# rlvc/FEALESS

Measured on AMD Instinct MI355X. Metric: frames/sec (640x480 RGB-D x N templates, 20 ICP iters), higher is better.
Workload: dtype u8

## Files before the change

fealess_amd/csrc/fl_icp.hip:

```cpp
#include "fl_internal.h"
#include <float.h>
#include <math.h>
#include <string.h>
#include <type_traits>
#include <mutex>
#include <map>
#include <utility>

#define ICP_BS_SMALL 256
#define ICP_BS_WIDE 1024
#define ICP_DT 512
#ifdef FL_ICP_PHASES
#define TSTAMP(k) do { if (threadIdx.x == 0) { long long now_ = clock64(); S.tacc[k] += now_ - S.tlast; S.tlast = now_; } } while (0)
#define CH_STAMP_BEGIN long long c_add = 0, c_bar = 0, c_last = clock64()
#define CH_STAMP(v) { const long long now_ = clock64(); v += now_ - c_last; c_last = now_; }
#define CH_STAMP_END(k) { if (threadIdx.x == 0) { S.hist[k] += (unsigned)(c_add >> 4); S.hist[(k) + 1] += (unsigned)(c_bar >> 4); } }
#define PR_STAMP_BARRIER(k, every) { const long long b0_ = clock64(); tile_barrier(); if (threadIdx.x == 64) S.hist[k] += (unsigned)(((clock64() - b0_) * (every)) >> 4); }
#define ST_STAMP_BEGIN long long st_acc[6] = {0, 0, 0, 0, 0, 0}, st_last = clock64()
#define ST_STAMP(k) { const long long now_ = clock64(); st_acc[k] += now_ - st_last; st_last = now_; }
#define ST_ARRIVED(a, b) asm volatile("" :: "v"(a), "v"(b));
#define ST_STAMP_END { if ((threadIdx.x & 63) == 0) for (int k = 0; k < 5; ++k) atomicAdd(&S.stime[k], (unsigned long long)st_acc[k]); }
#else
#define TSTAMP(k) do { } while (0)
#define CH_STAMP_BEGIN
#define CH_STAMP(v) { }
#define CH_STAMP_END(k) { }
#define PR_STAMP_BARRIER(k, every) tile_barrier()
#define ST_STAMP_BEGIN
#define ST_STAMP(k) { }
#define ST_ARRIVED(a, b)
#define ST_STAMP_END
#endif
__device__ __forceinline__ void tile_barrier()
{
  __builtin_amdgcn_s_waitcnt(0xC07F);
  __builtin_amdgcn_s_barrier();
}
#define ICP_PARITY_WPE 4
#define ICP_FAST_WPE 4
#define ICP_PLANE_WPE 4
#define ICP_MODE_WPE(MODE) ((MODE) == FL_ICP_PARITY ? ICP_PARITY_WPE : ((MODE) == FL_ICP_POINT_TO_PLANE ? ICP_PLANE_WPE : ICP_FAST_WPE))
#define ICP_NBQ 4
#define ICP_NBUF_SMALL 4
#define ICP_TILE_W 16
#define ICP_BMACRO 4
#define ICP_STAGE_CAP 384
#define ICP_NB 10

struct IcpWsLayout {
  size_t ref, mod, sref, zimg, nn, bnd, nd, dterm, perm, cell_start, cell_cur, nrm, total;
  int ncell_max;
};
static __host__ __device__ inline size_t al256(size_t v) { return (v + 255) & ~(size_t)255; }
static __host__ __device__ inline IcpWsLayout icp_layout(int n)
{
  IcpWsLayout L;
  size_t o = 0, nn = (size_t)(n > 0 ? n : 1);
  L.ncell_max = n + 4096;
  L.ref = o; o = al256(o + 12 * nn);
  L.mod = o; o = al256(o + 12 * nn);
  L.sref = o; o = al256(o + 16 * (nn + 4));
  L.zimg = o; o = al256(o + 4 * (nn + 4));
  L.nn = o; o = al256(o + 4 * nn);
  L.bnd = o; o = al256(o + 4 * nn);
  L.nd = o; o = al256(o + 4 * nn);
  L.dterm = o; o = al256(o + 4 * nn + 4 * ICP_DT);
  L.perm = o; o = al256(o + 4 * nn);
  L.cell_start = o; o = al256(o + 4 * ((size_t)L.ncell_max + 1));
  L.cell_cur = o; o = al256(o + 4 * (size_t)L.ncell_max);
  L.nrm = o; o = al256(o + 12 * nn);
  L.total = o;
  return L;
}
size_t fl_icp_ws_bytes(int n_pts_max) { return icp_layout(n_pts_max).total; }

struct IcpJob {
// ... 22 lines not shown
  const uint16_t *scene_base;
  size_t scene_stride;
  const FlPyrInfo *pyr;
  const int *class_first;
  const float *poses;
  const uint16_t *const *depth_ptrs;
  fl_recognition_result *results;
  const FlRefineJob *jobs;
  const int *order;
};

template <int BS_>
struct IcpSharedT {
  static constexpr int BS = BS_;
  static constexpr int NW = BS_ / 64;
  static constexpr int NPROD = NW >= 8 ? NW - NW / 4 : NW - 1;
  static constexpr int CHAIN_NBUF = BS_ >= 1024 ? 4 : ICP_NBUF_SMALL;
  static constexpr int TQ = NPROD * 64;
  int cw;
  __device__ __forceinline__ int producer_slot() const
  {
    const int t = (int)threadIdx.x, w = t >> 6;
    if (NW >= 8) return (w & 3) == 0 ? -1 : t - 64 * (1 + (w >> 2));
    const int v = (w - __builtin_amdgcn_readfirstlane(cw) - 1) & (NW - 1);
    return v == NW - 1 ? -1 : v * 64 + (t & 63);
  }
  __device__ __forceinline__ int chain_lane() const
  {
    const int t = (int)threadIdx.x;
    if (NW >= 8) return t < 64 ? t : -1;
    return (t >> 6) == __builtin_amdgcn_readfirstlane(cw) ? (t & 63) : -1;
  }
  static constexpr int TS = TQ + 4;
  float R[9], T[3], Ropt[9], Topt[3];
  float dist_mean, dist_diff, px, thr;
  int iter, n_corr, go, ok;
  int cnt, inl;
  int stop;
  int a1_next;
  float xmin, ymin, inv_c;
  int GX, GY, nsorted;
  float sums[16];
  double dsum[NW][32];
  int iscan[NW + 1];
  int iscan2[2][NW];
  float fred[4][NW];
  int n, rect_m[4], rect_r[4], status, g;
  alignas(16) float prod[2][15][TS];
  static constexpr bool BSUM = NW >= 8;
  alignas(16) float dtile[2][TQ];
  static constexpr int STAGE_FLOATS = NW * 384 * 4, TILE_FLOATS = 2 * 15 * TS + 2 * TQ;
  alignas(16) float stage_pad[STAGE_FLOATS > TILE_FLOATS ? STAGE_FLOATS - TILE_FLOATS : 4];
  alignas(16) float dchain[2][ICP_DT];
#ifdef FL_ICP_PHASES
  long long tacc[16], tlast, tkernel;
  long long wall0;
  unsigned long long stime[8];
  unsigned hist[40];
#endif
};

__device__ __forceinline__ bool vvalid(float z) { return z <= 900.0f; }
__device__ __forceinline__ float uniform_f(float v) { return __int_as_float(__builtin_amdgcn_readfirstlane(__float_as_int(v))); }
__device__ __forceinline__ int cvt_i32_sat(float f)
{
  int r;
  asm("v_cvt_i32_f32 %0, %1" : "=v"(r) : "v"(f));
  return r;
}

#include "fl_icp_search.h"

template <class SH>
__device__ __forceinline__ int block_sum_int(SH &S, int v)
{
#pragma unroll
  for (int s = 32; s >= 1; s >>= 1) v += __shfl_xor(v, s, 64);
  __syncthreads();
  if ((threadIdx.x & 63) == 0) S.iscan[threadIdx.x >> 6] = v;
  __syncthreads();
  int t = 0;
#pragma unroll
  for (int i = 0; i < SH::NW; ++i) t += S.iscan[i];
  return t;
}

__device__ __forceinline__ double shfl_xor_d(double v, int s)
{
  int lo = __double2loint(v), hi = __double2hiint(v);
  lo = __shfl_xor(lo, s, 64);
  hi = __shfl_xor(hi, s, 64);
  return __hiloint2double(hi, lo);
}

template <int NS, class SH>
__device__ __forceinline__ void block_sum_double(SH &S, double *v)
{
  const int lane = threadIdx.x & 63, wave = threadIdx.x >> 6;
#pragma unroll
  for (int k = 0; k < NS; ++k) {
    double x = v[k];
#pragma unroll
    for (int s = 32; s >= 1; s >>= 1) x += shfl_xor_d(x, s);
    v[k] = x;
  }
  __syncthreads();
  if (lane == 0)
    for (int k = 0; k < NS; ++k) S.dsum[wave][k] = v[k];
  __syncthreads();
  if (threadIdx.x < NS) {
    double t = 0;
// ... 418 lines not shown
  for (int a = 0; a < 6; ++a) A[a][a] += 1.0e-12 * tr;
  for (int c = 0; c < 6 && ok; ++c) {
    double d = A[c][c];
    for (int k = 0; k < c; ++k) d -= A[c][k] * A[c][k];
    if (!(d > 1.0e-13 * tr)) { ok = false; break; }
    d = sqrt(d);
    A[c][c] = d;
    for (int r = c + 1; r < 6; ++r) {
      double v = A[r][c];
      for (int k = 0; k < c; ++k) v -= A[r][k] * A[c][k];
      A[r][c] = v / d;
    }
  }
  if (ok) {
    for (int r = 0; r < 6; ++r) {
      double v = x[r];
      for (int k = 0; k < r; ++k) v -= A[r][k] * x[k];
      x[r] = v / A[r][r];
    }
    for (int r = 5; r >= 0; --r) {
      double v = x[r];
      for (int k = r + 1; k < 6; ++k) v -= A[k][r] * x[k];
      x[r] = v / A[r][r];
    }
    const double wx = x[0], wy = x[1], wz = x[2], t2 = wx * wx + wy * wy + wz * wz, t = sqrt(t2);
    const double sa = t > 1.0e-9 ? sin(t) / t : 1.0 - t2 / 6.0, sb = t > 1.0e-9 ? (1.0 - cos(t)) / t2 : 0.5 - t2 / 24.0;
    const double Kx[9] = {0, -wz, wy, wz, 0, -wx, -wy, wx, 0};
    for (int i = 0; i < 3; ++i)
      for (int j = 0; j < 3; ++j) {
        double k2 = 0;
        for (int k = 0; k < 3; ++k) k2 += Kx[i * 3 + k] * Kx[k * 3 + j];
        S.Ropt[i * 3 + j] = (float)((i == j ? 1.0 : 0.0) + sa * Kx[i * 3 + j] + sb * k2);
      }
    for (int k = 0; k < 3; ++k) S.Topt[k] = (float)x[3 + k];
  }
  S.ok = ok && finite_all(S.Ropt, 9) && finite_all(S.Topt, 3);
}
template <class SH>
__device__ __forceinline__ void pose_accumulate(SH &S)
{
  float RT[3];
  mat_vec(S.Ropt, S.T, RT);
  for (int k = 0; k < 3; ++k) S.T[k] = RT[k] + S.Topt[k];
  mat_mat(S.Ropt, S.R, S.R);
}
__device__ __forceinline__ void icp_result_none(fl_icp_result *res)
{
  for (int i = 0; i < 9; ++i) res->R[i] = 0.f;
  for (int i = 0; i < 3; ++i) res->T[i] = 0.f;
  res->dist_mean = -1.0f; res->px_ratio = 0.f;
  res->iters = 0; res->n_corr_last = 0;
}

template <class IDX>
__device__ __forceinline__ int nn_get(IDX v) { return sizeof(IDX) == 2 && (int)v == 0xFFFF ? -1 : (int)v; }
template <int MODE, bool ORG, class IDX, class SH>
__device__ __forceinline__ void icp_run(SH &S, uint8_t *wsb, const IcpWsLayout &L, int n_ref, int n_model,
                        int it_thr, float dmt, float ddt, fl_icp_result *res, const OrgGeom &og)
{
  constexpr int BS = SH::BS, NW = SH::NW;
  float *ref = (float *)(wsb + L.ref), *mod = (float *)(wsb + L.mod);
  float4 *sref = (float4 *)(wsb + L.sref);
  const float *jsrc = ORG ? (const float *)sref : ref;
  const int *idximg = ORG ? (const int *)((const uint8_t *)sref + org_idximg_offset(og.cw * og.ch)) : nullptr;
  constexpr bool IDX16 = sizeof(IDX) == 2;
  static_assert(!IDX16 || (MODE == FL_ICP_PARITY && ORG && SH::NW < 8), "16-bit indices: the 256-thread parity kernel of the organised search only");
  IDX *nn = (IDX *)(wsb + L.nn);
  bnd_t *bnd = (bnd_t *)(wsb + L.bnd);
  float *nd = (float *)(wsb + L.nd), *dterm = (float *)(wsb + L.dterm);
  const IDX *perm = (const IDX *)(wsb + L.perm);
  const uint16_t *pix = (const uint16_t *)(wsb + L.dterm);
  const float *zref = (const float *)(wsb + L.nd);
  const float *nrm = (const float *)(wsb + L.nrm);
  int *cell_start = (int *)(wsb + L.cell_start), *cell_cur = (int *)(wsb + L.cell_cur);
  constexpr bool plane = MODE == FL_ICP_POINT_TO_PLANE;
  constexpr int NSUM = plane ? 27 : 15;

  if (threadIdx.x == 0) {
    for (int i = 0; i < 9; ++i) S.R[i] = 0.f;
    for (int i = 0; i < 3; ++i) S.T[i] = 0.f;
    S.iter = 0;
    S.n_corr = 0;
    S.px = 0.f;
#ifdef FL_ICP_PHASES
    for (int i = 0; i < 16; ++i) S.tacc[i] = 0;
    for (int i = 0; i < 40; ++i) S.hist[i] = 0;
    for (int i = 0; i < 8; ++i) S.stime[i] = 0;
    S.tlast = clock64();
    S.tacc[6] = S.tlast - S.tkernel;
#endif
  }
  __syncthreads();
  if (n_model < 3 || n_ref < 3 || n_ref < n_model) {
    if (threadIdx.x == 0) icp_result_none(res);
    __syncthreads();
    return;
  }
  if (!ORG) build_grid(S, ref, n_ref, sref, cell_start, cell_cur, L.ncell_max);
  TSTAMP(0);
  for (int i = threadIdx.x; i < n_model; i += BS)
    if (!vvalid(mod[3 * i + 2])) { mod[3 * i] = 0.f; mod[3 * i + 1] = 0.f; mod[3 * i + 2] = 0.f; }
  if (threadIdx.x == 0) {
    S.R[0] = S.R[4] = S.R[8] = 1.f;
    S.dist_diff = FLT_MAX;
  }
  __syncthreads();
  constexpr bool SPEC = BS >= ICP_BS_WIDE && MODE == FL_ICP_PARITY && ORG;
  static_assert(!(IDX16 && SPEC), "pix[] / zref[] live where the deferred chain keeps dterm[] / nd[]");
  float mean_ub = l2dist_phase<MODE, SPEC, false>(S, mod, ref, bnd, dterm, n_model, FLT_MAX, nullptr, nullptr, pix, zref, og);
  int pending = SPEC ? 1 : 0;
  bool have_nn = false;
  float old_mean = 0.0f;

  const auto ctx = org_search_ctx(mod, bnd, perm, (const float *)sref, (const float *)(wsb + L.zimg), n_model, og);
  auto chain_and_search = [&](const int pend, const bool want, const float r_lim, const float old_mean_) {
    if (pend && threadIdx.x < 64) {
      const float acc = chain_deferred<SH::CHAIN_NBUF>(dterm, S.dchain, n_model);
      if (threadIdx.x == 0) {
        const int counter = S.cnt, inl = S.inl;
        float dm = acc;
        if (counter > 0) dm /= (float)inl;
        const float new_mean = counter > 0 ? dm : FLT_MAX;
        S.px = counter > 0 ? (float)inl / (float)counter : 0.0f;
        if (pend == 2) {
          S.dist_diff = old_mean_ - new_mean;
          pose_accumulate(S);
        }
        S.dist_mean = new_mean;
        const bool go = (new_mean > dmt) && (S.dist_diff > ddt) && (S.iter < it_thr);
        *(volatile int *)&S.stop = go ? 0 : 1;
      }
    }
    if (want)
      org_search<SH, SPEC>(S, ctx, r_lim, true, [&](bool active, int i, float, float, float, int j, float d) {
        if (active) {
          nn[i] = (IDX)j;
          nd[i] = d;
          if (j >= 0) bnd_st(bnd, i, sqrt_upper(d));
        }
      });
  };

  for (;;) {
    if (SPEC) {
      const int it_done = __builtin_amdgcn_readfirstlane(S.iter);
      const bool want = !have_nn && it_done >= 1 && it_done < it_thr;
      if (pending || want) {
        const float r_lim = pending ? sqrtf(3.0f * mean_ub) * 1.00001f : sqrtf(3 * S.dist_mean);
        if (threadIdx.x == 0) { S.a1_next = 0; S.stop = 0; }
        __syncthreads();
        chain_and_search(pending, want, uniform_f(r_lim), old_mean);
        __syncthreads();
        TSTAMP(2);
        if (want) have_nn = true;
        pending = 0;
      }
    }
    if (threadIdx.x == 0) S.go = (S.dist_mean > dmt) && (S.dist_diff > ddt) && (S.iter < it_thr);
    __syncthreads();
    if (!S.go) break;
    if (threadIdx.x == 0) { ++S.iter; S.thr = plane ? (3 * S.dist_mean) * (3 * S.dist_mean) : 3 * S.dist_mean; S.a1_next = 0; }
    __syncthreads();
// ... 18 lines not shown
#pragma unroll
          for (int b = a; b < 6; ++b) ds[q++] += J[a] * J[b];
#pragma unroll
        for (int a = 0; a < 6; ++a) ds[21 + a] += J[a] * e;
      } else if (!parity) {
        const float m[3] = {m0, m1, m2}, r[3] = {r0, r1, r2};
#pragma unroll
        for (int a = 0; a < 3; ++a)
#pragma unroll
          for (int b = 0; b < 3; ++b) ds[a * 3 + b] += (double)m[a] * (double)r[b];
#pragma unroll
        for (int q = 0; q < 3; ++q) { ds[9 + q] += (double)m[q]; ds[12 + q] += (double)r[q]; }
      }
    };
    if (!index_pairs && !SPEC) {
      const float r_thr = uniform_f(sqrtf(thr));
      auto on_found = [&](bool active, int i, float qx, float qy, float qz, int j, float d) {
        const bool keep = d <= thr;
        if (active) {
          nn[i] = (IDX)(keep ? j : -1);
          if (j >= 0) bnd_st(bnd, i, sqrt_upper(d));
        }
        if (keep) {
          ++kept;
          if (!parity) { const F3 rv = ld3_u32(jsrc, j); pair_sums(qx, qy, qz, rv.x, rv.y, rv.z, j); }
        }
      };
      if (ORG) {
        if (MODE == FL_ICP_PARITY && NW < 8) org_search_pipe(S, ctx, r_thr, on_found);
        else org_search<SH, SPEC>(S, ctx, r_thr, false, on_found);
      } else {
        const NnGrid G = nn_grid(S);
        int i = threadIdx.x;
        float qx = 0.f, qy = 0.f, qz = 0.f, qb = 0.f;
        if (i < n_model) { const F3 q3 = ld3_u32(mod, i); qx = q3.x; qy = q3.y; qz = q3.z; qb = bnd_ld(bnd, i); }
        for (; i < n_model; i += BS) {
          const int in = min(i + BS, n_model - 1);
          const F3 nq3 = ld3_u32(mod, in);
          const float nqx = nq3.x, nqy = nq3.y, nqz = nq3.z, nqb = bnd_ld(bnd, in);
          int j = -1;
          float d = NAN;
          if (thr >= 0.f && isfinite(qx) && isfinite(qy) && isfinite(qz))
            nn_search_grid(G, sref, cell_start, qx, qy, qz, nn_radius(qx, qy, qz, fminf(qb, r_thr)), &j, &d);
          on_found(true, i, qx, qy, qz, j, d);
          qx = nqx; qy = nqy; qz = nqz; qb = nqb;
        }
      }
      __syncthreads();
      TSTAMP(2);
    }
    constexpr int TQ = parity ? SH::TQ : BS;
    const int slot = parity ? S.producer_slot() : (int)threadIdx.x;
    const int clane = parity ? S.chain_lane() : -1;
    const int ntiles = (parity || index_pairs) ? (rows + TQ - 1) / TQ : 0;
    float acc = 0.0f;
    if (parity && iter > 1) {
      struct Row {
        int j;
        float d;
        bool in;
        F3 m, r;
      };
      constexpr bool ZIMG = ORG && NW < 8;
      const float *zimg = (const float *)(wsb + L.zimg);
      const float inv_cw = uniform_f(1.0f / (float)max(og.cw, 1));
      auto row_load = [&](Row &w, int t) {
        const int i = t * TQ + slot;
        w.in = i < rows;
        const int ic = min(i, rows - 1);
        w.j = ld_u32(nn, ic);
        w.d = SPEC ? ld_u32(nd, ic) : 0.0f;
        w.m = ld3_u32(mod, ic);
      };
      auto row_gather = [&](Row &w) {
        if (!(w.in && (!SPEC || w.d <= thr)) || (IDX16 && w.j == 0xFFFF)) w.j = -1;
        if (ZIMG) w.r.x = ld_u32(zimg, max(w.j, 0));
        else w.r = ld3_u32(jsrc, max(w.j, 0));
      };
      auto row_write = [&](const Row &w, int t) {
        const bool have = w.j >= 0;
        if (SPEC && have) ++kept;
        float (*tile)[SH::TS] = S.prod[t & 1];
        F3 rp = w.r;
        if (ZIMG) {
          const int jj = max(w.j, 0);
          int vv, uu;
          if (ctx.small_crop) {
            vv = (int)(((float)jj + 0.5f) * inv_cw);
            uu = jj - __mul24(vv, og.cw);
            if (uu < 0) { --vv; uu += og.cw; } else if (uu >= og.cw) { ++vv; uu -= og.cw; }
          } else {
            vv = jj / og.cw;
            uu = jj - vv * og.cw;
          }
          rp = org_point(og, uu, vv, w.r.x);
        }
        const float mm[3] = {have ? w.m.x : 0.0f, have ? w.m.y : 0.0f, have ? w.m.z : 0.0f};
        const float rr[3] = {have ? rp.x : 0.0f, have ? rp.y : 0.0f, have ? rp.z : 0.0f};
#pragma unroll
        for (int a = 0; a < 3; ++a)
#pragma unroll
          for (int b = 0; b < 3; ++b) tile[a * 3 + b][slot] = mm[a] * rr[b];
#pragma unroll
        for (int q = 0; q < 3; ++q) { tile[9 + q][slot] = mm[q]; tile[12 + q][slot] = rr[q]; }
      };
      const bool chain_wave = __builtin_amdgcn_readfirstlane(clane) >= 0;
      if (chain_wave) {
        CH_STAMP_BEGIN;
        for (int t = 0; t < ntiles; ++t) {
          if (t > 0 && clane < 15)
            acc = chain_tile<SH::CHAIN_NBUF>(S.prod[(t - 1) & 1][clane], min(TQ, rows - (t - 1) * TQ), acc);
          CH_STAMP(c_add);
          tile_barrier();
          CH_STAMP(c_bar);
        }
        CH_STAMP_END(22);
      } else if (slot >= 0) {
        Row X, Y, Z;
        row_load(X, 0);
        row_load(Y, 1);
        row_gather(X);
        for (int t = 0; t < ntiles; t += 3) {
          row_load(Z, t + 2); row_gather(Y); row_write(X, t);
          PR_STAMP_BARRIER(24, 3);
          if (t + 1 < ntiles) {
            row_load(X, t + 3); row_gather(Z); row_write(Y, t + 1);
            tile_barrier();
          }
          if (t + 2 < ntiles) {
            row_load(Y, t + 4); row_gather(X); row_write(Z, t + 2);
            tile_barrier();
          }
        }
      } else {
        for (int t = 0; t < ntiles; ++t) tile_barrier();
      }
      __syncthreads();
    } else
    for (int t = 0; t < ntiles; ++t) {
      if (slot >= 0) {
        const int i = t * TQ + slot;
        float m[3] = {0.f, 0.f, 0.f}, r[3] = {0.f, 0.f, 0.f};
        bool have_m = false, have_pair = false;
        if (i < rows) {
          if (iter == 1) {
            if (i < n_model) {
              have_m = true;
              have_pair = true;
              if (vvalid(mod[3 * i + 2])) { m[0] = mod[3 * i]; m[1] = mod[3 * i + 1]; m[2] = mod[3 * i + 2]; }
            }
            if (vvalid(ref[3 * i + 2])) { r[0] = ref[3 * i]; r[1] = ref[3 * i + 1]; r[2] = ref[3 * i + 2]; }
          } else {
            const int j = nn_get(nn[i]);
            if (j >= 0) {
              have_m = have_pair = true;
              m[0] = mod[3 * i]; m[1] = mod[3 * i + 1]; m[2] = mod[3 * i + 2];
              r[0] = jsrc[3 * j]; r[1] = jsrc[3 * j + 1]; r[2] = jsrc[3 * j + 2];
            }
          }
        }
        if (parity) {
          float (*tile)[SH::TS] = S.prod[t & 1];
#pragma unroll
          for (int a = 0; a < 3; ++a)
#pragma unroll
            for (int b = 0; b < 3; ++b) tile[a * 3 + b][slot] = have_pair ? m[a] * r[b] : 0.0f;
#pragma unroll
          for (int q = 0; q < 3; ++q) { tile[9 + q][slot] = have_m ? m[q] : 0.0f; tile[12 + q][slot] = r[q]; }
        } else {
#pragma unroll
          for (int a = 0; a < 3; ++a)
#pragma unroll
            for (int b = 0; b < 3; ++b) ds[a * 3 + b] += (double)m[a] * (double)r[b] * (have_pair ? 1.0 : 0.0);
#pragma unroll
          for (int q = 0; q < 3; ++q) { ds[9 + q] += have_m ? (double)m[q] : 0.0; ds[12 + q] += (double)r[q]; }
        }
      } else if (t > 0 && clane >= 0 && clane < 15) {
        acc = chain_tile<SH::CHAIN_NBUF>(S.prod[(t - 1) & 1][clane], min(TQ, rows - (t - 1) * TQ), acc);
      }
      if (parity) __syncthreads();
    }
    if (parity && ntiles > 0 && clane >= 0 && clane < 15)
      acc = chain_tile<SH::CHAIN_NBUF>(S.prod[(ntiles - 1) & 1][clane], min(TQ, rows - (ntiles - 1) * TQ), acc);
    kept = block_sum_int(S, kept);
    TSTAMP(3);
    const int ncm = index_pairs ? n_model : kept, ncr = index_pairs ? n_ref : kept;
    if (threadIdx.x == 0) S.n_corr = ncm;
    if (ncr < 3 || ncm < 3) {
      __syncthreads();
      if (threadIdx.x == 0) S.iter = it_thr;
      __syncthreads();
      continue;
    }
    if (MODE == FL_ICP_PARITY) {
      if (clane >= 0 && clane < 15) S.sums[clane] = acc;
      __syncthreads();
    } else {
      double dd[NSUM];
#pragma unroll
      for (int k = 0; k < NSUM; ++k) dd[k] = (double)ds[k];
      block_sum_double<NSUM>(S, dd);
    }
    if (threadIdx.x == 0) {
      if (plane) solve_point_to_plane(S);
      else solve_rigid<MODE>(S, ncm, ncr);
    }
    __syncthreads();
    TSTAMP(4);
    if (!S.ok) continue;
    float Ro[9], To[3];
    for (int k = 0; k < 9; ++k) Ro[k] = S.Ropt[k];
    for (int k = 0; k < 3; ++k) To[k] = S.Topt[k];
    old_mean = S.dist_mean;
    __syncthreads();
    mean_ub = l2dist_phase<MODE, SPEC, IDX16>(S, mod, ref, bnd, dterm, n_model, 3 * old_mean, Ro, To, pix, zref, og);
    TSTAMP(5);
    if (SPEC) {
      pending = 2;
      have_nn = false;
      continue;
    }
    if (threadIdx.x == 0) {
      S.dist_diff = old_mean - S.dist_mean;
      pose_accumulate(S);
    }
    __syncthreads();
  }
  if (threadIdx.x == 0) {
    for (int i = 0; i < 9; ++i) res->R[i] = S.R[i];
    for (int i = 0; i < 3; ++i) res->T[i] = S.T[i];
    res->dist_mean = S.dist_mean;
    res->px_ratio = S.px;
    res->iters = S.iter;
    res->n_corr_last = S.n_corr;
#ifdef FL_ICP_PHASES
    for (int i = 0; i < 6; ++i) res->R[i] = (float)S.tacc[i];
    res->R[6] = (float)S.tacc[6];
    res->R[7] = (float)(clock64() - S.tkernel);
// ... 96 lines not shown
        scene_normal(scene, a.w, a.h, rr[0] + p % cw, rr[1] + p / cw, a.fx, a.fy, a.cx, a.cy, nv);
        nrm[3 * k] = nv[0]; nrm[3 * k + 1] = nv[1]; nrm[3 * k + 2] = nv[2];
      }
    }
    kept_before += total;
  }
  if (threadIdx.x < 3 * NN_OVERRUN) rimg[3 * np + threadIdx.x] = INFINITY;
  if (zimg && threadIdx.x < NN_OVERRUN + 1) zimg[np + threadIdx.x] = NAN;
  __syncthreads();
  return kept_before;
}

template <class SH, class IDX>
__device__ __forceinline__ void build_tile_order(SH &S, const int *idximg, int cw, int ch, int n, IDX *perm)
{
  constexpr int BS = SH::BS, NW = SH::NW;
  int *cnt = (int *)&S.prod[0][0][0];
  constexpr int CAP = (int)(sizeof(S.prod) / 4);
  constexpr int TW = ICP_TILE_W, TH = 64 / ICP_TILE_W;
  static_assert(TW * TH == 64 && (TW & (TW - 1)) == 0, "a tile is one wavefront of pixels");
  const int ntx = (cw + TW - 1) / TW, nty = (ch + TH - 1) / TH, ntile = ntx * nty;
  if (ntile > CAP) {
    if constexpr (sizeof(IDX) == 2) {
      for (unsigned i = threadIdx.x; i < (unsigned)n; i += BS) {
        unsigned o = 2 * i;
        asm volatile("" : "+v"(o));
        *(IDX *)((char *)perm + (size_t)o) = (IDX)i;
      }
    } else {
      for (int i = threadIdx.x; i < n; i += BS) perm[i] = i;
    }
    __syncthreads();
    return;
  }
  const int lane = threadIdx.x & 63, wv = threadIdx.x >> 6;
  const float inv_ntx = 1.0f / (float)ntx;
  auto tile_index = [&](int t, bool &has) {
    const int ty = (int)(((float)t + 0.5f) * inv_ntx);
    int tx = t - ty * ntx;
    if (ty & 1) tx = ntx - 1 - tx;
    const int c = lane / TH, x = tx * TW + ((ty & 1) ? TW - 1 - c : c), y = ty * TH + (lane & (TH - 1));
    int k = NN_IDX_NONE;
    if (x < cw && y < ch) k = idximg[y * cw + x];
    has = (unsigned)k < (unsigned)NN_IDX_NONE;
    return k;
  };
  for (int t = wv; t < ntile; t += NW) {
    bool has;
    tile_index(t, has);
    const unsigned long long bal = __ballot(has);
    if (lane == 0) cnt[t] = __popcll(bal);
  }
  __syncthreads();
  {
    const int per = (ntile + BS - 1) / BS, lo = min((int)threadIdx.x * per, ntile), hi = min(lo + per, ntile);
    int mine = 0;
    for (int t = lo; t < hi; ++t) mine += cnt[t];
    int inc = mine;
#pragma unroll
    for (int d = 1; d < 64; d <<= 1) {
      const int v = __shfl_up(inc, d, 64);
      if (lane >= d) inc += v;
    }
    if (lane == 63) S.iscan[wv] = inc;
    __syncthreads();
    int before = 0;
#pragma unroll
    for (int w = 0; w < NW; ++w) before += w < wv ? S.iscan[w] : 0;
    int ex = before + inc - mine;
    for (int t = lo; t < hi; ++t) { const int c = cnt[t]; cnt[t] = ex; ex += c; }
  }
  __syncthreads();
  for (int t = wv; t < ntile; t += NW) {
    bool has;
    const int k = tile_index(t, has);
    const unsigned long long bal = __ballot(has);
    if (has) perm[cnt[t] + __builtin_amdgcn_mbcnt_hi((unsigned)(bal >> 32), __builtin_amdgcn_mbcnt_lo((unsigned)bal, 0u))] = (IDX)k;
  }
  __syncthreads();
}

#define ICP_WPE(MODE, BS) ((BS) == ICP_BS_SMALL ? ICP_MODE_WPE(MODE) : (BS) / 256)

template <int MODE, int BS>
__global__ __launch_bounds__(BS) void k_icp_clouds(IcpArgs a)
{
  extern __shared__ __align__(16) uint8_t icp_smem[];
  using SH = IcpSharedT<BS>;
  SH &S = *(SH *)icp_smem;
  const IcpWsLayout L = icp_layout(a.n_max);
  uint8_t *wsb = a.ws + (size_t)blockIdx.x * a.ws_stride;
  const OrgGeom none = {};
  if (threadIdx.x == 0) S.cw = 0;
  __syncthreads();
  icp_run<MODE, false, int>(S, wsb, L, a.job.n_ref, a.job.n_model, a.it_thr, a.dmt, a.ddt, &a.results[blockIdx.x].det.icp, none);
}

template <int MODE, int BS, int WPE = ICP_WPE(MODE, BS), class IDX = int>
__global__ __launch_bounds__(BS) __attribute__((amdgpu_waves_per_eu(WPE, WPE > 4 ? WPE : 4)))
void k_icp_pipeline(IcpArgs a)
{
  extern __shared__ __align__(16) uint8_t icp_smem[];
  using SH = IcpSharedT<BS>;
  SH &S = *(SH *)icp_smem;
#ifdef FL_ICP_PHASES
  if (threadIdx.x == 0) { S.tkernel = clock64(); S.wall0 = wall_clock64(); }
#endif
  const int job = a.order ? a.order[blockIdx.x] : (int)blockIdx.x, rank = a.job.kind == 0 && !a.jobs ? job % a.ranks : 0;
  const int frame = a.job.kind == 0 ? (a.jobs ? a.jobs[job].frame : job / a.ranks) : job;
  const IcpWsLayout L = icp_layout(a.n_max);
  uint8_t *wsb = a.ws + (size_t)job * a.ws_stride;
  float *ref = (float *)(wsb + L.ref), *mod = (float *)(wsb + L.mod);

  fl_recognition_result *res = &a.results[job];
  if (a.job.kind == 0 && a.jobs && frame < 0) return;
  const uint16_t *scene, *model;
  float r_match[9], t_match[3];
  bool model_01mm;
  if (a.job.kind == 1) {
    if (threadIdx.x == 0) {
      for (int k = 0; k < 4; ++k) { S.rect_m[k] = a.job.rect_model[k]; S.rect_r[k] = a.job.rect_ref[k]; }
      S.status = FL_OK;
      res->status = FL_OK;
      res->found = 1;
    }
    scene = a.job.scene_depth;
    model = a.job.model_depth;
    for (int k = 0; k < 9; ++k) r_match[k] = a.job.r_match[k];
    for (int k = 0; k < 3; ++k) t_match[k] = a.job.t_match[k];
    model_01mm = false;
    __syncthreads();
  } else {
    const uint8_t *fws = a.frame_ws + (size_t)frame * a.frame_stride;
    const int *counters = (const int *)(fws + a.off_count);
    const fl_match *matches = (const fl_match *)(fws + a.off_match);
    if (threadIdx.x == 0) {
      S.status = FL_OK;
      S.g = -1;
      res->n_matches = a.jobs ? 1 : counters[1];
      res->found = 0;
      res->status = FL_OK;
      if (!a.jobs && counters[2]) S.status = res->status = FL_ERR_OVERFLOW;
      else if (a.jobs || counters[1] > rank) {
        const fl_match best = a.jobs ? a.jobs[job].match : matches[rank];
        res->best = best;
        const int g = a.class_first[best.class_idx] + best.template_id;
        const FlPyrInfo pi = a.pyr[g];
        S.g = g;
        S.rect_m[0] = pi.off_x0; S.rect_m[1] = pi.off_y0; S.rect_m[2] = pi.width0; S.rect_m[3] = pi.height0;
        S.rect_r[0] = best.x; S.rect_r[1] = best.y; S.rect_r[2] = pi.width0; S.rect_r[3] = pi.height0;
        if (!a.depth_ptrs[g]) S.status = res->status = FL_ERR_STATE;
      }
    }
    __syncthreads();
    if (S.g < 0 || S.status != FL_OK) return;
    const int g = S.g;
    scene = (const uint16_t *)((const uint8_t *)a.scene_base + (size_t)frame * a.scene_stride);
    model = a.depth_ptrs[g];
    const float *p = a.poses + 13 * (size_t)g;
    for (int i = 0; i < 3; ++i) {
      for (int j = 0; j < 3; ++j) r_match[i * 3 + j] = p[i * 4 + j];
      t_match[i] = p[i * 4 + 3];
    }
    model_01mm = true;
  }
  {
    const int *rm = S.rect_m, *rr = S.rect_r;
    const bool bad = rm[0] < 0 || rm[1] < 0 || rm[2] < 0 || rm[3] < 0 || rm[0] + rm[2] > a.w || rm[1] + rm[3] > a.h ||
                     rr[0] < 0 || rr[1] < 0 || rr[2] < 0 || rr[3] < 0 || rr[0] + rr[2] > a.w || rr[1] + rr[3] > a.h ||
                     rm[2] != rr[2] || rm[3] != rr[3] || (long long)rm[2] * rm[3] > a.n_max;
    if (bad) {
      if (threadIdx.x == 0) { res->status = FL_ERR_ASSERT; res->det.status = FL_ERR_ASSERT; res->found = 0; }
      return;
    }
  }
  if (threadIdx.x == 0) S.cw = 0;
  __syncthreads();
  float *rimg = (float *)(wsb + L.sref);
  const int np = crop_clouds(S, a, scene, model, model_01mm, S.rect_m, S.rect_r, ref, mod,
                             MODE == FL_ICP_POINT_TO_PLANE ? (float *)(wsb + L.nrm) : nullptr, rimg,
                             (int *)((uint8_t *)rimg + org_idximg_offset(S.rect_m[2] * S.rect_m[3])),
                             MODE == FL_ICP_PARITY && BS < ICP_BS_WIDE ? (float *)(wsb + L.zimg) : nullptr,
                             sizeof(IDX) == 2 ? (uint16_t *)(wsb + L.dterm) : nullptr, (float *)(wsb + L.nd));
  const OrgGeom og = {__builtin_amdgcn_readfirstlane(S.rect_r[2]), __builtin_amdgcn_readfirstlane(S.rect_r[3]),
                      uniform_f((float)S.rect_r[0] - a.cx), uniform_f((float)S.rect_r[1] - a.cy), a.fx, a.fy,
                      __builtin_amdgcn_readfirstlane(S.rect_r[0]), __builtin_amdgcn_readfirstlane(S.rect_r[1]), a.cx, a.cy,
                      uniform_f(1.0f / a.fx), uniform_f(1.0f / a.fy)};
  build_tile_order(S, (const int *)((const uint8_t *)rimg + org_idximg_offset(og.cw * og.ch)), og.cw, og.ch, np, (IDX *)(wsb + L.perm));
  float mc[3] = {0, 0, 0}, rc[3] = {0, 0, 0};
  if (MODE == FL_ICP_PARITY) {
    {
      constexpr int TQ = SH::TQ;
      const int slot = S.producer_slot(), clane = S.chain_lane(), ntiles = (np + TQ - 1) / TQ;
      float acc = 0.0f;
      for (int t = 0; t < ntiles; ++t) {
        if (slot >= 0) {
          const int i = t * TQ + slot;
          F3 m3 = {0.f, 0.f, 0.f}, r3 = {0.f, 0.f, 0.f};
          if (i < np) { m3 = ld3_u32(mod, i); r3 = ld3_u32(ref, i); }
          float (*tile)[SH::TS] = S.prod[t & 1];
          tile[0][slot] = m3.x; tile[1][slot] = m3.y; tile[2][slot] = m3.z;
          tile[3][slot] = r3.x; tile[4][slot] = r3.y; tile[5][slot] = r3.z;
        } else if (t > 0 && clane >= 0 && clane < 6) {
          acc = chain_tile<SH::CHAIN_NBUF>(S.prod[(t - 1) & 1][clane], min(TQ, np - (t - 1) * TQ), acc);
        }
        __syncthreads();
      }
      if (ntiles > 0 && clane >= 0 && clane < 6)
        acc = chain_tile<SH::CHAIN_NBUF>(S.prod[(ntiles - 1) & 1][clane], min(TQ, np - (ntiles - 1) * TQ), acc);
      if (clane >= 0 && clane < 6) S.sums[clane] = acc;
    }
    __syncthreads();
    for (int k = 0; k < 3; ++k) { mc[k] = S.sums[k]; rc[k] = S.sums[3 + k]; }
    if (np > 0)
      for (int k = 0; k < 3; ++k) { mc[k] /= (float)np; rc[k] /= (float)np; }
  } else {
    double ds[6] = {0, 0, 0, 0, 0, 0};
    for (int i = threadIdx.x; i < np; i += BS)
      for (int k = 0; k < 3; ++k) { ds[k] += mod[3 * i + k]; ds[3 + k] += ref[3 * i + k]; }
    block_sum_double<6>(S, ds);
    if (np > 0)
      for (int k = 0; k < 3; ++k) { mc[k] = (float)(S.dsum[0][k] / np); rc[k] = (float)(S.dsum[0][3 + k] / np); }
  }
  float t_tmp[3], t_init[3];
  for (int k = 0; k < 3; ++k) { t_tmp[k] = rc[k] - mc[k]; t_init[k] = t_tmp[k] + t_match[k]; }
  __syncthreads();
  for (int i = threadIdx.x; i < np; i += BS) {
    if (!vvalid(mod[3 * i + 2])) continue;
    const float I[9] = {1, 0, 0, 0, 1, 0, 0, 0, 1};
    float v[3] = {mod[3 * i], mod[3 * i + 1], mod[3 * i + 2]}, o[3];
    mat_vec(I, v, o);
    mod[3 * i] = o[0] + t_tmp[0];
    mod[3 * i + 1] = o[1] + t_tmp[1];
    mod[3 * i + 2] = o[2] + t_tmp[2];
  }
  __syncthreads();
  icp_run<MODE, true, IDX>(S, wsb, L, np, np, a.it_thr, a.dmt, a.ddt, &res->det.icp, og);
  if (threadIdx.x == 0) {
    const fl_icp_result &ic = res->det.icp;
    float Rt[3];
    mat_vec(ic.R, t_init, Rt);
    for (int k = 0; k < 3; ++k) res->det.T_final[k] = Rt[k] + ic.T[k];
    mat_mat(ic.R, r_match, res->det.R_final);
    res->det.n_points = np;
    res->det.status = FL_OK;
    for (int i = 0; i < 3; ++i) {
      for (int j = 0; j < 3; ++j) res->pose[i * 4 + j] = res->det.R_final[i * 3 + j];
      res->pose[i * 4 + 3] = res->det.T_final[i];
    }
    res->pose[12] = res->pose[13] = res->pose[14] = 0.f;
    res->pose[15] = 1.f;
    res->found = 1;
#ifdef FL_ICP_PHASES
    for (int i = 0; i < 16; ++i) res->pose[i] = (float)S.hist[i];
    for (int i = 0; i < 9; ++i) res->det.R_final[i] = (float)S.hist[16 + i];
    for (int i = 0; i < 3; ++i) res->det.T_final[i] = (float)S.hist[26 + i];
    for (int i = 0; i < 5; ++i) res->pose[11 + i] = (float)S.stime[i];
    {
      const long long w1 = wall_clock64();
      res->pose[0] = (float)((S.wall0 >> 24) & 0xffffff); res->pose[1] = (float)(S.wall0 & 0xffffff);
      res->pose[2] = (float)((w1 >> 24) & 0xffffff); res->pose[3] = (float)(w1 & 0xffffff);
      unsigned hwid;
      asm volatile("s_getreg_b32 %0, hwreg(HW_REG_HW_ID)" : "=s"(hwid));
      res->pose[4] = (float)(hwid & 0xffffff);
    }
#endif
  }
}

__global__ __launch_bounds__(256) void k_depth_to_3d(const uint16_t *__restrict__ depth, int w, int h, float fx, float fy,
                                                     float cx, float cy, float *__restrict__ out)
{
  const int x = blockIdx.x * 64 + (threadIdx.x & 63), y = blockIdx.y * 4 + (threadIdx.x >> 6);
  if (x >= w || y >= h) return;
  const float inv_fx = 1.0f / fx, inv_fy = 1.0f / fy;
  const unsigned d = depth[(size_t)y * w + x];
  const float z = d == 0 ? NAN : (float)d * (float)(1 / 1000.0);
  float *p = out + ((size_t)y * w + x) * 3;
  p[0] = (((float)x - cx) * inv_fx) * z;
  p[1] = (((float)y - cy) * inv_fy) * z;
  p[2] = z;
}

extern "C" int fl_depth_to_3d(fl_context *ctx, const uint16_t *depth, int w, int h, double fx, double fy, double cx,
                              double cy, float *out, int mem)
{
  if (!ctx || !depth || !out || w <= 0 || h <= 0) return FL_ERR_INVALID;
  FL_HIP(ctx, hipSetDevice(ctx->device));
  const size_t nin = (size_t)w * h * 2, nout = (size_t)w * h * 12;
  const uint16_t *din = depth;
  float *dout = out;
  if (mem == FL_MEM_HOST) {
    void *s = nullptr;
    int rc = fl_scratch(ctx, fl_align(nin, 256) + nout, &s);
    if (rc) return rc;
    FL_HIP(ctx, hipMemcpyAsync(s, depth, nin, hipMemcpyHostToDevice, ctx->stream));
    din = (const uint16_t *)s;
    dout = (float *)((uint8_t *)s + fl_align(nin, 256));
  }
  dim3 grid((w + 63) / 64, (h + 3) / 4);
  hipLaunchKernelGGL(k_depth_to_3d, grid, dim3(256), 0, ctx->stream, din, w, h, (float)fx, (float)fy, (float)cx, (float)cy,
                     dout);
  FL_HIP(ctx, hipGetLastError());
  if (mem == FL_MEM_HOST) {
    FL_HIP(ctx, hipMemcpyAsync(out, dout, nout, hipMemcpyDeviceToHost, ctx->stream));
    FL_HIP(ctx, hipStreamSynchronize(ctx->stream));
  }
  return FL_OK;
}

__global__ __launch_bounds__(256) void k_icp_count(IcpArgs a, int *__restrict__ size)
{
  __shared__ int part[4];
  const int job = blockIdx.x;
  const uint8_t *fws = a.frame_ws + (size_t)job * a.frame_stride;
  const int *counters = (const int *)(fws + a.off_count);
  const fl_match *matches = (const fl_match *)(fws + a.off_match);
  int n = 0;
// ... 19 lines not shown
  __syncthreads();
  if (threadIdx.x == 0) size[job] = part[0] + part[1] + part[2] + part[3];
}

#define ICP_ORDER_MAX 8192
__global__ __launch_bounds__(1024) void k_icp_order(const int *__restrict__ size, int n, int *__restrict__ order)
{
  extern __shared__ unsigned long long okeys[];
  int m = 1;
  while (m < n) m <<= 1;
  for (int i = threadIdx.x; i < m; i += 1024)
    okeys[i] = i < n ? ((unsigned long long)(unsigned)(0x7fffffff - size[i]) << 32) | (unsigned)i : ~0ull;
  __syncthreads();
  for (int k = 2; k <= m; k <<= 1)
    for (int j = k >> 1; j > 0; j >>= 1) {
      for (int i = threadIdx.x; i < m; i += 1024) {
        const int l = i ^ j;
        if (l > i) {
          const unsigned long long x = okeys[i], y = okeys[l];
          if (((i & k) == 0) == (x > y)) { okeys[i] = y; okeys[l] = x; }
        }
      }
      __syncthreads();
    }
  for (int i = threadIdx.x; i < n; i += 1024) order[i] = (int)(unsigned)(okeys[i] & 0xffffffffull);
}

#define ICP_WPE_MAX 5
static_assert(sizeof(IcpSharedT<ICP_BS_SMALL>) + 16 <= 160 * 1024 / ICP_WPE_MAX, "IcpSharedT<256> must leave room for 5 workgroups per CU");
static_assert(sizeof(IcpSharedT<ICP_BS_WIDE>) + 16 <= 160 * 1024, "IcpSharedT<1024> must fit the CU's LDS");
template <int BS, typename K>
static int icp_launch_one(fl_context *ctx, K kern, int n_jobs, const IcpArgs &a)
{
  size_t lds = (sizeof(IcpSharedT<BS>) + 15) & ~(size_t)15;
  const long cap = ctx->opt.icp_wg_per_cu;
  if (BS == ICP_BS_SMALL && cap >= 1 && cap <= 3) {
    const size_t want = ((size_t)(160 * 1024) / (size_t)cap - 256) & ~(size_t)15;
    if (want > lds) lds = want;
  }
  {
    static std::mutex mu;
    static std::map<std::pair<const void *, int>, size_t> attr_set;
    std::lock_guard<std::mutex> lock(mu);
    size_t &cur = attr_set[{(const void *)kern, ctx->device}];
    if (cur < lds) {
      size_t attr = lds > (size_t)(82 * 1024) ? lds : (size_t)(82 * 1024);
      if (attr > (size_t)(160 * 1024)) attr = (size_t)(160 * 1024);
      FL_HIP(ctx, hipFuncSetAttribute((const void *)kern, hipFuncAttributeMaxDynamicSharedMemorySize, (int)attr));
      cur = attr;
    }
  }
  hipLaunchKernelGGL(kern, dim3(n_jobs), dim3(BS), lds, ctx->stream, a);
  FL_HIP(ctx, hipGetLastError());
  return FL_OK;
}
static bool icp_wide(fl_context *ctx, int n_jobs)
{
  if (ctx->opt.icp_wide == 0) return false;
  if (ctx->opt.icp_wide == 1) return true;
  return n_jobs <= 2 * ctx->cus;
}
static int icp_small_wpe(fl_context *ctx, int n_jobs)
{
  if (ctx->opt.icp_occ == 4 || ctx->opt.icp_occ == 5) return (int)ctx->opt.icp_occ;
  const int cus = ctx->cus;
  const int r4 = (n_jobs + 4 * cus - 1) / (4 * cus), r5 = (n_jobs + 5 * cus - 1) / (5 * cus);
  return 1.25 * r5 < 1.0 * r4 ? 5 : 4;
}
static bool icp_idx16(fl_context *ctx, const IcpArgs &a)
{
  return ctx->opt.icp_idx16 != 0 && a.n_max <= 65535;
}
template <int MODE>
static int icp_launch_mode(fl_context *ctx, int n_jobs, const IcpArgs &a)
{
  const bool wide = icp_wide(ctx, n_jobs);
  if constexpr (MODE == FL_ICP_PARITY) {
    if (a.job.kind != 2 && !wide) {
      const bool five = icp_small_wpe(ctx, n_jobs) == 5;
      if (icp_idx16(ctx, a))
        return five ? icp_launch_one<ICP_BS_SMALL>(ctx, k_icp_pipeline<MODE, ICP_BS_SMALL, 5, uint16_t>, n_jobs, a)
                    : icp_launch_one<ICP_BS_SMALL>(ctx, k_icp_pipeline<MODE, ICP_BS_SMALL, ICP_PARITY_WPE, uint16_t>, n_jobs, a);
      if (five) return icp_launch_one<ICP_BS_SMALL>(ctx, k_icp_pipeline<MODE, ICP_BS_SMALL, 5>, n_jobs, a);
    }
  }
  if (a.job.kind == 2)
    return wide ? icp_launch_one<ICP_BS_WIDE>(ctx, k_icp_clouds<MODE, ICP_BS_WIDE>, n_jobs, a)
                : icp_launch_one<ICP_BS_SMALL>(ctx, k_icp_clouds<MODE, ICP_BS_SMALL>, n_jobs, a);
  return wide ? icp_launch_one<ICP_BS_WIDE>(ctx, k_icp_pipeline<MODE, ICP_BS_WIDE>, n_jobs, a)
              : icp_launch_one<ICP_BS_SMALL>(ctx, k_icp_pipeline<MODE, ICP_BS_SMALL>, n_jobs, a);
}
static int icp_launch(fl_context *ctx, int n_jobs, const IcpArgs &a)
{
  switch (a.mode) {
    case FL_ICP_PARITY: return icp_launch_mode<FL_ICP_PARITY>(ctx, n_jobs, a);
    case FL_ICP_FAST: return icp_launch_mode<FL_ICP_FAST>(ctx, n_jobs, a);
    case FL_ICP_POINT_TO_PLANE: return icp_launch_mode<FL_ICP_POINT_TO_PLANE>(ctx, n_jobs, a);
    default: return fl_set_error(ctx, FL_ERR_INVALID, "unknown fl_icp_mode");
  }
}

static IcpArgs icp_args(uint8_t *ws, int n_max, int it_thr, float dmt, float ddt, int mode)
{
  IcpArgs a;
  memset(&a, 0, sizeof(a));
  a.ws = ws;
// ... 226 lines not shown
```

Measured before the change: 94300.

## Fuse pre-translation, invalid-point zeroing and first distance pass into one pipelined pass

For the 256-thread parity kernel, a new first_pass applies the initial translation, zeros invalid model points, computes the initial distances and bounds, and accumulates the iteration-1 cross-covariance sums through the producer/chain tile pipeline, all in one sweep over the model and reference clouds. Iteration 1 then reuses these stored sums instead of re-reading the clouds and re-running the tile reduction. This removes two separate passes over the model plus a redundant summation pass. The fused path adds code complexity, carries a new shared-memory array, and the instrumentation is compiled only under FL_ICP_PHASES.

```diff
diff --git a/fealess_amd/csrc/fl_icp.hip b/fealess_amd/csrc/fl_icp.hip
--- a/fealess_amd/csrc/fl_icp.hip
+++ b/fealess_amd/csrc/fl_icp.hip
@@ -12,6 +12,7 @@
 #define ICP_DT 512
 #ifdef FL_ICP_PHASES
 #define TSTAMP(k) do { if (threadIdx.x == 0) { long long now_ = clock64(); S.tacc[k] += now_ - S.tlast; S.tlast = now_; } } while (0)
+#define SSTAMP(k) do { if (threadIdx.x == 0) { long long now_ = clock64(); S.tset[k] += now_ - S.tslast; S.tslast = now_; } } while (0)
 #define CH_STAMP_BEGIN long long c_add = 0, c_bar = 0, c_last = clock64()
 #define CH_STAMP(v) { const long long now_ = clock64(); v += now_ - c_last; c_last = now_; }
 #define CH_STAMP_END(k) { if (threadIdx.x == 0) { S.hist[k] += (unsigned)(c_add >> 4); S.hist[(k) + 1] += (unsigned)(c_bar >> 4); } }
@@ -22,6 +23,7 @@
 #define ST_STAMP_END { if ((threadIdx.x & 63) == 0) for (int k = 0; k < 5; ++k) atomicAdd(&S.stime[k], (unsigned long long)st_acc[k]); }
 #else
 #define TSTAMP(k) do { } while (0)
+#define SSTAMP(k) do { } while (0)
 #define CH_STAMP_BEGIN
 #define CH_STAMP(v) { }
 #define CH_STAMP_END(k) { }
@@ -150,11 +152,13 @@
   static constexpr int STAGE_FLOATS = NW * 384 * 4, TILE_FLOATS = 2 * 15 * TS + 2 * TQ;
   alignas(16) float stage_pad[STAGE_FLOATS > TILE_FLOATS ? STAGE_FLOATS - TILE_FLOATS : 4];
   alignas(16) float dchain[2][ICP_DT];
+  float first_sums[16];
 #ifdef FL_ICP_PHASES
   long long tacc[16], tlast, tkernel;
   long long wall0;
   unsigned long long stime[8];
   unsigned hist[40];
+  long long tset[10], tslast;
 #endif
 };
 
@@ -679,11 +683,109 @@
   res->iters = 0; res->n_corr_last = 0;
 }
 
+template <class SH>
+__device__ __forceinline__ void first_pass(SH &S, float *mod, const float *ref, bnd_t *bnd, int n, const float *pre_t)
+{
+  constexpr int TQ = SH::TQ;
+  const int slot = S.producer_slot(), clane = S.chain_lane();
+  const int ntiles = (n + TQ - 1) / TQ;
+  const float thr = FLT_MAX;
+  int counter = 0, inl = 0;
+  float acc = 0.0f;
+  struct Row { F3 m, r; };
+  auto row_load = [&](Row &w, int t) {
+    const int i = min(t * TQ + slot, n - 1);
+    w.m = ld3_u32(mod, i);
+    w.r = ld3_u32(ref, i);
+  };
+  auto row_process = [&](const Row &w, int t) {
+    const int i = t * TQ + slot;
+    float m[3] = {0.f, 0.f, 0.f}, r[3] = {0.f, 0.f, 0.f}, term = 0.0f;
+    if (i < n) {
+      float a[3] = {w.m.x, w.m.y, w.m.z};
+      if (vvalid(a[2])) {
+        const float I[9] = {1, 0, 0, 0, 1, 0, 0, 0, 1};
+        float o[3];
+        mat_vec(I, a, o);
+        a[0] = o[0] + pre_t[0];
+        a[1] = o[1] + pre_t[1];
+        a[2] = o[2] + pre_t[2];
+      }
+      if (!vvalid(a[2])) { a[0] = 0.f; a[1] = 0.f; a[2] = 0.f; }
+      mod[3 * i] = a[0];
+      mod[3 * i + 1] = a[1];
+      mod[3 * i + 2] = a[2];
+      const float b0 = w.r.x, b1 = w.r.y, b2 = w.r.z;
+      const float ex = a[0] - b0, ey = a[1] - b1, ez = a[2] - b2;
+      bnd_st(bnd, i, sqrt_upper(ex * ex + ey * ey + ez * ez));
+      if (vvalid(b2) && vvalid(a[2])) {
+        const float dx = a[0] - b0, dy = a[1] - b1, dz = a[2] - b2;
+        const float dist = (float)sqrt((double)dx * dx + (double)dy * dy + (double)dz * dz);
+        if (dist <= thr) { term = dist; ++inl; }
+        ++counter;
+      }
+      if (vvalid(a[2])) { m[0] = a[0]; m[1] = a[1]; m[2] = a[2]; }
+      if (vvalid(b2)) { r[0] = b0; r[1] = b1; r[2] = b2; }
+    }
+    float (*tile)[SH::TS] = S.prod[t & 1];
+#pragma unroll
+    for (int p = 0; p < 3; ++p)
+#pragma unroll
+      for (int q = 0; q < 3; ++q) tile[p * 3 + q][slot] = m[p] * r[q];
+#pragma unroll
+    for (int q = 0; q < 3; ++q) { tile[9 + q][slot] = m[q]; tile[12 + q][slot] = r[q]; }
+    S.dtile[t & 1][slot] = term;
+  };
+  auto chain_step = [&](int t) {
+    const float *col = clane < 15 ? S.prod[t & 1][clane] : S.dtile[t & 1];
+    acc = chain_tile<SH::CHAIN_NBUF>(col, min(TQ, n - t * TQ), acc);
+  };
+  const bool chain_wave = __builtin_amdgcn_readfirstlane(clane) >= 0;
+  if (chain_wave) {
+    for (int t = 0; t < ntiles; ++t) {
+      if (t > 0 && clane < 16) chain_step(t - 1);
+      tile_barrier();
+    }
+  } else if (slot >= 0) {
+    Row A, B;
+    row_load(A, 0);
+    for (int t = 0; t < ntiles; t += 2) {
+      row_load(B, t + 1);
+      row_process(A, t);
+      tile_barrier();
+      if (t + 1 < ntiles) {
+        row_load(A, t + 2);
+        row_process(B, t + 1);
+        tile_barrier();
+      }
+    }
+  }
+  __syncthreads();
+  if (chain_wave && clane < 16) chain_step(ntiles - 1);
+  counter = block_sum_int(S, counter);
+  inl = block_sum_int(S, inl);
+  if (clane >= 0 && clane < 15) S.first_sums[clane] = acc;
+  if (clane == 15) S.sums[0] = acc;
+  __syncthreads();
+  float dm = S.sums[0];
+  if (counter > 0) dm /= (float)inl;
+  if (threadIdx.x == 0) {
+    if (counter > 0) {
+      S.dist_mean = dm;
+      S.px = (float)inl / (float)counter;
+    } else {
+      S.dist_mean = FLT_MAX;
+      S.px = 0.0f;
+    }
+  }
+  __syncthreads();
+}
+
 template <class IDX>
 __device__ __forceinline__ int nn_get(IDX v) { return sizeof(IDX) == 2 && (int)v == 0xFFFF ? -1 : (int)v; }
-template <int MODE, bool ORG, class IDX, class SH>
+template <int MODE, bool ORG, class IDX, bool FIRST = false, class SH>
 __device__ __forceinline__ void icp_run(SH &S, uint8_t *wsb, const IcpWsLayout &L, int n_ref, int n_model,
-                        int it_thr, float dmt, float ddt, fl_icp_result *res, const OrgGeom &og)
+                        int it_thr, float dmt, float ddt, fl_icp_result *res, const OrgGeom &og, const float *pre_t = nullptr)
 {
   constexpr int BS = SH::BS, NW = SH::NW;
   float *ref = (float *)(wsb + L.ref), *mod = (float *)(wsb + L.mod);
@@ -725,16 +827,23 @@
   }
   if (!ORG) build_grid(S, ref, n_ref, sref, cell_start, cell_cur, L.ncell_max);
   TSTAMP(0);
-  for (int i = threadIdx.x; i < n_model; i += BS)
-    if (!vvalid(mod[3 * i + 2])) { mod[3 * i] = 0.f; mod[3 * i + 1] = 0.f; mod[3 * i + 2] = 0.f; }
+  SSTAMP(9);
+  if (!FIRST)
+    for (int i = threadIdx.x; i < n_model; i += BS)
+      if (!vvalid(mod[3 * i + 2])) { mod[3 * i] = 0.f; mod[3 * i + 1] = 0.f; mod[3 * i + 2] = 0.f; }
   if (threadIdx.x == 0) {
     S.R[0] = S.R[4] = S.R[8] = 1.f;
     S.dist_diff = FLT_MAX;
   }
   __syncthreads();
+  SSTAMP(5);
   constexpr bool SPEC = BS >= ICP_BS_WIDE && MODE == FL_ICP_PARITY && ORG;
   static_assert(!(IDX16 && SPEC), "pix[] / zref[] live where the deferred chain keeps dterm[] / nd[]");
-  float mean_ub = l2dist_phase<MODE, SPEC, false>(S, mod, ref, bnd, dterm, n_model, FLT_MAX, nullptr, nullptr, pix, zref, og);
+  static_assert(!FIRST || (MODE == FL_ICP_PARITY && ORG && !SPEC), "first_pass: the 256-thread parity pipeline kernel only");
+  float mean_ub = 0.0f;
+  if constexpr (FIRST) first_pass(S, mod, ref, bnd, n_model, pre_t);
+  else mean_ub = l2dist_phase<MODE, SPEC, false>(S, mod, ref, bnd, dterm, n_model, FLT_MAX, nullptr, nullptr, pix, zref, og);
+  SSTAMP(6);
   int pending = SPEC ? 1 : 0;
   bool have_nn = false;
   float old_mean = 0.0f;
@@ -859,8 +968,10 @@
     constexpr int TQ = parity ? SH::TQ : BS;
     const int slot = parity ? S.producer_slot() : (int)threadIdx.x;
     const int clane = parity ? S.chain_lane() : -1;
-    const int ntiles = (parity || index_pairs) ? (rows + TQ - 1) / TQ : 0;
+    const bool summed = FIRST && iter == 1;
+    const int ntiles = ((parity || index_pairs) && !summed) ? (rows + TQ - 1) / TQ : 0;
     float acc = 0.0f;
+    SSTAMP(9);
     if (parity && iter > 1) {
       struct Row {
         int j;
@@ -944,7 +1055,7 @@
       }
       __syncthreads();
     } else
-    for (int t = 0; t < ntiles; ++t) {
+    for (int t = 0; t < (FIRST ? 0 : ntiles); ++t) {
       if (slot >= 0) {
         const int i = t * TQ + slot;
         float m[3] = {0.f, 0.f, 0.f}, r[3] = {0.f, 0.f, 0.f};
@@ -989,8 +1100,10 @@
     }
     if (parity && ntiles > 0 && clane >= 0 && clane < 15)
       acc = chain_tile<SH::CHAIN_NBUF>(S.prod[(ntiles - 1) & 1][clane], min(TQ, rows - (ntiles - 1) * TQ), acc);
+    if (summed && clane >= 0 && clane < 15) acc = S.first_sums[clane];
     kept = block_sum_int(S, kept);
     TSTAMP(3);
+    if (iter == 1) SSTAMP(7);
     const int ncm = index_pairs ? n_model : kept, ncr = index_pairs ? n_ref : kept;
     if (threadIdx.x == 0) S.n_corr = ncm;
     if (ncr < 3 || ncm < 3) {
@@ -1193,6 +1306,7 @@
     if (lane == 0) cnt[t] = __popcll(bal);
   }
   __syncthreads();
+  SSTAMP(1);
   {
     const int per = (ntile + BS - 1) / BS, lo = min((int)threadIdx.x * per, ntile), hi = min(lo + per, ntile);
     int mine = 0;
@@ -1219,8 +1333,12 @@
     if (has) perm[cnt[t] + __builtin_amdgcn_mbcnt_hi((unsigned)(bal >> 32), __builtin_amdgcn_mbcnt_lo((unsigned)bal, 0u))] = (IDX)k;
   }
   __syncthreads();
-}
-
+  SSTAMP(2);
+}
+
+#ifdef FL_ICP_PHASES
+__device__ unsigned long long g_icp_setup[12];
+#endif
 #define ICP_WPE(MODE, BS) ((BS) == ICP_BS_SMALL ? ICP_MODE_WPE(MODE) : (BS) / 256)
 
 template <int MODE, int BS>
@@ -1245,8 +1363,13 @@
   using SH = IcpSharedT<BS>;
   SH &S = *(SH *)icp_smem;
 #ifdef FL_ICP_PHASES
-  if (threadIdx.x == 0) { S.tkernel = clock64(); S.wall0 = wall_clock64(); }
+  if (threadIdx.x == 0) {
+    S.tkernel = clock64(); S.wall0 = wall_clock64();
+    for (int i = 0; i < 10; ++i) S.tset[i] = 0;
+    S.tslast = S.tkernel;
+  }
 #endif
+  constexpr bool FIRST = MODE == FL_ICP_PARITY && BS == ICP_BS_SMALL;
   const int job = a.order ? a.order[blockIdx.x] : (int)blockIdx.x, rank = a.job.kind == 0 && !a.jobs ? job % a.ranks : 0;
   const int frame = a.job.kind == 0 ? (a.jobs ? a.jobs[job].frame : job / a.ranks) : job;
   const IcpWsLayout L = icp_layout(a.n_max);
@@ -1318,11 +1441,13 @@
   if (threadIdx.x == 0) S.cw = 0;
   __syncthreads();
   float *rimg = (float *)(wsb + L.sref);
+  SSTAMP(9);
   const int np = crop_clouds(S, a, scene, model, model_01mm, S.rect_m, S.rect_r, ref, mod,
                              MODE == FL_ICP_POINT_TO_PLANE ? (float *)(wsb + L.nrm) : nullptr, rimg,
                              (int *)((uint8_t *)rimg + org_idximg_offset(S.rect_m[2] * S.rect_m[3])),
                              MODE == FL_ICP_PARITY && BS < ICP_BS_WIDE ? (float *)(wsb + L.zimg) : nullptr,
                              sizeof(IDX) == 2 ? (uint16_t *)(wsb + L.dterm) : nullptr, (float *)(wsb + L.nd));
+  SSTAMP(0);
   const OrgGeom og = {__builtin_amdgcn_readfirstlane(S.rect_r[2]), __builtin_amdgcn_readfirstlane(S.rect_r[3]),
                       uniform_f((float)S.rect_r[0] - a.cx), uniform_f((float)S.rect_r[1] - a.cy), a.fx, a.fy,
                       __builtin_amdgcn_readfirstlane(S.rect_r[0]), __builtin_amdgcn_readfirstlane(S.rect_r[1]), a.cx, a.cy,
@@ -1366,17 +1491,20 @@
   float t_tmp[3], t_init[3];
   for (int k = 0; k < 3; ++k) { t_tmp[k] = rc[k] - mc[k]; t_init[k] = t_tmp[k] + t_match[k]; }
   __syncthreads();
-  for (int i = threadIdx.x; i < np; i += BS) {
-    if (!vvalid(mod[3 * i + 2])) continue;
-    const float I[9] = {1, 0, 0, 0, 1, 0, 0, 0, 1};
-    float v[3] = {mod[3 * i], mod[3 * i + 1], mod[3 * i + 2]}, o[3];
-    mat_vec(I, v, o);
-    mod[3 * i] = o[0] + t_tmp[0];
-    mod[3 * i + 1] = o[1] + t_tmp[1];
-    mod[3 * i + 2] = o[2] + t_tmp[2];
-  }
-  __syncthreads();
-  icp_run<MODE, true, IDX>(S, wsb, L, np, np, a.it_thr, a.dmt, a.ddt, &res->det.icp, og);
+  SSTAMP(3);
+  if (!FIRST)
+    for (int i = threadIdx.x; i < np; i += BS) {
+      if (!vvalid(mod[3 * i + 2])) continue;
+      const float I[9] = {1, 0, 0, 0, 1, 0, 0, 0, 1};
+      float v[3] = {mod[3 * i], mod[3 * i + 1], mod[3 * i + 2]}, o[3];
+      mat_vec(I, v, o);
+      mod[3 * i] = o[0] + t_tmp[0];
+      mod[3 * i + 1] = o[1] + t_tmp[1];
+      mod[3 * i + 2] = o[2] + t_tmp[2];
+    }
+  __syncthreads();
+  SSTAMP(4);
+  icp_run<MODE, true, IDX, FIRST>(S, wsb, L, np, np, a.it_thr, a.dmt, a.ddt, &res->det.icp, og, FIRST ? t_tmp : nullptr);
   if (threadIdx.x == 0) {
     const fl_icp_result &ic = res->det.icp;
     float Rt[3];
@@ -1405,6 +1533,9 @@
       asm volatile("s_getreg_b32 %0, hwreg(HW_REG_HW_ID)" : "=s"(hwid));
       res->pose[4] = (float)(hwid & 0xffffff);
     }
+    for (int i = 0; i < 10; ++i) atomicAdd(&g_icp_setup[i], (unsigned long long)S.tset[i]);
+    atomicAdd(&g_icp_setup[10], (unsigned long long)(clock64() - S.tkernel));
+    atomicAdd(&g_icp_setup[11], 1ull);
 #endif
   }
 }
@@ -1530,6 +1661,20 @@
   }
   hipLaunchKernelGGL(kern, dim3(n_jobs), dim3(BS), lds, ctx->stream, a);
   FL_HIP(ctx, hipGetLastError());
+#ifdef FL_ICP_PHASES
+  {
+    unsigned long long h[12], zero[12] = {};
+    FL_HIP(ctx, hipStreamSynchronize(ctx->stream));
+    FL_HIP(ctx, hipMemcpyFromSymbol(h, HIP_SYMBOL(g_icp_setup), sizeof(h)));
+    FL_HIP(ctx, hipMemcpyToSymbol(HIP_SYMBOL(g_icp_setup), zero, sizeof(zero)));
+    if (h[11]) {
+      const double w = (double)h[11];
+      fprintf(stderr, "icp set-up cycles per workgroup (%llu workgroups, life %.0f): crop %.0f, tile counts %.0f, tile placing %.0f, getMean %.0f, "
+              "pre-translation %.0f, copyPoints %.0f, initial distances / first pass %.0f, iteration 1 sums %.0f, between %.0f\n", h[11], h[10] / w,
+              h[0] / w, h[1] / w, h[2] / w, h[3] / w, h[4] / w, h[5] / w, h[6] / w, h[7] / w, h[9] / w);
+    }
+  }
+#endif
   return FL_OK;
 }
 static bool icp_wide(fl_context *ctx, int n_jobs)
```

After: 95860, median of 6. +1.7%, better.
